# intel/neural-compressor

Measured on AMD Instinct MI355X. Metric: llama2_7b_gptq_int4_g128_quantize_wall_clock, lower is better.
Workload: dtype bf16

## Files before the change

### include/inc_mi355x.h

```cpp
#ifndef INC_MI355X_H_
#define INC_MI355X_H_

#include <stdint.h>

#ifdef __cplusplus
extern "C" {
#endif

#define INC_OK 0
#define INC_ERR_BAD_ARG (-1)
#define INC_ERR_UNSUPPORTED (-2)
#define INC_ERR_LAUNCH (-3)
#define INC_ERR_WORKSPACE (-4)

#define INC_F32 0
#define INC_F16 1
#define INC_BF16 2

#define INC_SCHEME_ASYM 0
#define INC_SCHEME_SYM 1

typedef void* inc_stream_t;

int inc_abi_version(void);
// ... 184 lines not shown
                          inc_stream_t stream);
int inc_sq_weight_col_absmax(const void* w, int wdtype, int64_t N, int64_t K, float* out, inc_stream_t stream);
int inc_sq_cal_scale(const float* amax_x, const float* amax_w, int64_t K, float alpha, float weight_max_lb, float* scale,
                     inc_stream_t stream);
int inc_sq_quant_weight(const void* w, int wdtype, int64_t N, int64_t K, int64_t Kp, const float* smooth, int8_t* qw,
                        float* w_scale, int32_t* rowsum, inc_stream_t stream);
int inc_sq_quant_act(const void* x, int xdtype, int64_t M, int64_t K, int64_t Kp, const float* in_scale, float sx, float zp,
                     int8_t* out, inc_stream_t stream);
int inc_w8a8_gemm(const int8_t* xq, const int8_t* wq, const float* alpha, const int32_t* corr, const void* bias, void* y,
                  int ydtype, int64_t M, int64_t N, int64_t K, void* workspace, int64_t workspace_bytes,
                  inc_stream_t stream);
int inc_sq_quant_act_token(const void* x, int xdtype, int64_t M, int64_t K, int64_t Kp, const float* in_scale, int8_t* xq,
                           float* row_scale, inc_stream_t stream);
int inc_w8a8_gemm_rowscale(const int8_t* xq, const int8_t* wq, const float* row_scale, const float* alpha, const void* bias,
                           void* y, int ydtype, int64_t M, int64_t N, int64_t K, void* workspace, int64_t workspace_bytes,
                           inc_stream_t stream);

#define INC_MX_FP8_E4M3 0
#define INC_MX_FP4_E2M1 4
#define INC_MX_KTILE 128
#define INC_MX_GEMV_MAX_M 16
int inc_mx_quant(const void* x, int xdtype, int64_t M, int64_t K, int64_t Kp, int fmt, uint8_t* codes, uint8_t* scales,
                 inc_stream_t stream);
int inc_mx_gemm(const uint8_t* xq, const uint8_t* xs, int xfmt, const uint8_t* wq, const uint8_t* ws, int wfmt, const void* bias,
                void* y, int ydtype, int64_t M, int64_t N, int64_t Kp, inc_stream_t stream);
int inc_mx_gemv(const uint8_t* xq, const uint8_t* xs, int xfmt, const uint8_t* wq, const uint8_t* ws, int wfmt, const void* bias,
                void* y, int ydtype, int64_t M, int64_t N, int64_t Kp, inc_stream_t stream);
int inc_mx_gemv_multi(int n, const uint8_t* xq, const uint8_t* xs, int xfmt, const uint8_t* const* wq, const uint8_t* const* ws,
                      int wfmt, const void* const* bias, void* const* y, int ydtype, int64_t M, const int64_t* N, int64_t Kp,
                      inc_stream_t stream);
int inc_mx_moe_gemm(int mode, const uint8_t* aq, const uint8_t* as, int afmt, const int32_t* route, const uint8_t* wq,
                    const uint8_t* ws, int wfmt, const void* routing_weights, int wdtype, void* out, int odtype, int64_t T, int top_k,
                    int64_t E, int64_t N, int64_t Kp, inc_stream_t stream);

int inc_fp8_quant_rows(const void* x, int xdtype, int64_t M, int64_t K, int64_t Kp, const float* in_scale, uint8_t* codes,
                       float* row_scale, inc_stream_t stream);
int inc_fp8_gemm(const uint8_t* xq, const float* row_scale, const uint8_t* wq, const float* alpha, const void* bias, void* y, int ydtype,
                 int64_t M, int64_t N, int64_t Kp, inc_stream_t stream);
int inc_fp8_gemv(const uint8_t* xq, const float* row_scale, const uint8_t* wq, const float* alpha, const void* bias, void* y, int ydtype,
                 int64_t M, int64_t N, int64_t Kp, inc_stream_t stream);
int inc_fp8_moe_gemm(int mode, const uint8_t* aq, const float* a_scale, const int32_t* route, const uint8_t* wq, const float* alpha,
                     const void* routing_weights, int wdtype, void* out, int odtype, int64_t T, int top_k, int64_t E, int64_t N,
                     int64_t Kp, inc_stream_t stream);

int inc_probe_hbm_triad(float* a, const float* b, const float* c, float s, int64_t n, inc_stream_t stream);
int inc_probe_hbm_copy(void* dst, const void* src, int64_t bytes, int variant, inc_stream_t stream);
int inc_probe_mfma_bf16(const void* src, float* sink, int blocks, int iters, double* flops_out, inc_stream_t stream);
int inc_trace_marker(int id, inc_stream_t stream);

int inc_fwd_silu_mul(const void* gate, const void* up, void* out, int64_t n, int dtype, inc_stream_t stream);
int inc_fwd_rope(const void* q, const void* k, const void* cos, const void* sin, void* q_out, void* k_out, int64_t B, int64_t Hq,
                 int64_t Hk, int64_t T, int64_t D, const int64_t* strides, int64_t cs_batch, int dtype, inc_stream_t stream);
int inc_fwd_rmsnorm(const void* x, const void* w, void* out, int64_t rows, int64_t cols, float eps, int dtype, inc_stream_t stream);

#ifdef __cplusplus
}
#endif
#endif
```

### neural_compressor_amd/_lib.py

```python

import ctypes
import os
from ctypes import c_char_p, c_float, c_int, c_int64, c_void_p

_HERE = os.path.dirname(os.path.abspath(__file__))
LIB_PATH = os.path.join(_HERE, "libinc_mi355x.so")
ABI_VERSION = 12

INC_OK = 0
INC_F32, INC_F16, INC_BF16 = 0, 1, 2
INC_SCHEME_ASYM, INC_SCHEME_SYM = 0, 1

_P = c_void_p
SIGNATURES = {
    "inc_abi_version": (c_int, []),
    "inc_error_string": (c_char_p, [c_int]),
    "inc_target_arch": (c_char_p, []),
    "inc_pack_rows": (c_int, [_P, _P, c_int64, c_int64, c_int, c_int, _P]),
    "inc_unpack_rows": (c_int, [_P, _P, c_int64, c_int64, c_int, c_int, c_int, _P]),
    "inc_woq_pack": (c_int, [_P, c_int, _P, _P, _P, _P, _P, c_int64, c_int64, c_int64, c_int, c_int, _P]),
    "inc_woq_unpack": (c_int, [_P, _P, _P, _P, c_int64, c_int64, c_int64, c_int, _P, _P, _P]),
    "inc_woq_dequant": (c_int, [_P, _P, _P, _P, _P, c_int, c_int64, c_int64, c_int64, c_int, c_int, _P]),
    "inc_dequant_ints": (c_int, [_P, _P, c_int, _P, _P, _P, c_int, c_int64, c_int64, c_int64, c_int, _P]),
    "inc_woq_gemm_workspace_bytes": (c_int64, [c_int64, c_int64, c_int64]),
# ... 53 lines not shown
    "inc_gptq_find_params": (
        c_int,
        [_P, c_int64, c_int64, c_int64, c_int, c_int, c_int, c_int, _P, _P, c_int64, c_int64, _P],
    ),
    "inc_sq_channel_minmax": (c_int, [_P, c_int, c_int64, c_int64, c_int64, _P, _P, _P]),
    "inc_sq_weight_col_absmax": (c_int, [_P, c_int, c_int64, c_int64, _P, _P]),
    "inc_sq_cal_scale": (c_int, [_P, _P, c_int64, c_float, c_float, _P, _P]),
    "inc_sq_quant_weight": (c_int, [_P, c_int, c_int64, c_int64, c_int64, _P, _P, _P, _P, _P]),
    "inc_sq_quant_act": (c_int, [_P, c_int, c_int64, c_int64, c_int64, _P, c_float, c_float, _P, _P]),
    "inc_w8a8_gemm_workspace_bytes": (c_int64, [c_int64, c_int64, c_int64]),
    "inc_w8a8_gemm": (c_int, [_P, _P, _P, _P, _P, _P, c_int, c_int64, c_int64, c_int64, _P, c_int64, _P]),
    "inc_sq_quant_act_token": (c_int, [_P, c_int, c_int64, c_int64, c_int64, _P, _P, _P, _P]),
    "inc_w8a8_gemm_rowscale": (c_int, [_P, _P, _P, _P, _P, _P, c_int, c_int64, c_int64, c_int64, _P, c_int64, _P]),
    "inc_mx_quant": (c_int, [_P, c_int, c_int64, c_int64, c_int64, c_int, _P, _P, _P]),
    "inc_mx_gemm": (c_int, [_P, _P, c_int, _P, _P, c_int, _P, _P, c_int, c_int64, c_int64, c_int64, _P]),
    "inc_mx_gemv": (c_int, [_P, _P, c_int, _P, _P, c_int, _P, _P, c_int, c_int64, c_int64, c_int64, _P]),
    "inc_mx_gemv_multi": (c_int, [c_int, _P, _P, c_int, _P, _P, c_int, _P, _P, c_int, c_int64, _P, c_int64, _P]),
    "inc_mx_moe_gemm": (
        c_int,
        [c_int, _P, _P, c_int, _P, _P, _P, c_int, _P, c_int, _P, c_int, c_int64, c_int, c_int64, c_int64, c_int64, _P],
    ),
    "inc_fp8_quant_rows": (c_int, [_P, c_int, c_int64, c_int64, c_int64, _P, _P, _P, _P]),
    "inc_fp8_gemm": (c_int, [_P, _P, _P, _P, _P, _P, c_int, c_int64, c_int64, c_int64, _P]),
    "inc_fp8_gemv": (c_int, [_P, _P, _P, _P, _P, _P, c_int, c_int64, c_int64, c_int64, _P]),
    "inc_fp8_moe_gemm": (
        c_int,
        [c_int, _P, _P, _P, _P, _P, _P, c_int, _P, c_int, c_int64, c_int, c_int64, c_int64, c_int64, _P],
    ),
    "inc_awq_repack": (c_int, [_P, _P, c_int64, c_int64, c_int64, c_int, _P, _P, _P]),
    "inc_gptq_find_params_mse": (
        c_int,
        [_P, c_int64, c_int64, c_int64, c_int, c_int, c_int, c_int, c_int, c_float, c_float, _P, _P, c_int64, c_int64, _P],
    ),
    "inc_gptq_quant_block": (
        c_int,
        [_P, _P, _P, _P, _P, _P, c_int, _P, c_int64, c_int64, c_int64, c_int64, c_int, c_int, c_int, _P],
    ),
    "inc_gptq_quant_block_params": (c_int, [_P, _P, _P, _P, _P, _P, c_int, _P, c_int64, c_int64, c_int64, c_int64, c_int, c_int, c_int, c_int, _P]),
    "inc_gptq_lazy_update": (c_int, [_P, _P, _P, c_int64, c_int64, c_int64, c_int, _P]),
    "inc_gptq_lazy_update_cols": (c_int, [_P, _P, _P, c_int64, c_int64, c_int64, c_int, c_int64, c_int64, _P]),
    "inc_probe_hbm_triad": (c_int, [_P, _P, _P, c_float, c_int64, _P]),
    "inc_probe_hbm_copy": (c_int, [_P, _P, c_int64, c_int, _P]),
    "inc_probe_mfma_bf16": (c_int, [_P, _P, c_int, c_int, _P, _P]),
    "inc_trace_marker": (c_int, [c_int, _P]),
    "inc_gptq_quantize_layer": (c_int, [_P, _P, _P, _P, c_int64, _P, _P, c_int64, _P, _P, c_int, _P, c_int64, c_int64, c_int, c_int, c_int,
                                        c_int, c_int, c_int, _P, _P]),
    "inc_chol_diag_block": (c_int, [_P, c_int64, c_int, _P, c_int64, _P, c_int, _P]),
    "inc_gptq_inverse_factor_workspace_bytes": (c_int64, [c_int64, c_int]),
    "inc_gptq_inverse_factor": (c_int, [_P, c_int64, _P, _P, c_int64, _P, c_int, _P, _P]),
    "inc_awq_act_abs_sum": (c_int, [_P, c_int, c_int64, c_int64, _P, _P]),
    "inc_awq_weight_scale_workspace_bytes": (c_int64, [c_int64, c_int64, c_int]),
    "inc_awq_weight_scale": (c_int, [_P, c_int, c_int64, c_int64, c_int, _P, _P, c_int64, _P]),
    "inc_fwd_silu_mul": (c_int, [_P, _P, _P, c_int64, c_int, _P]),
    "inc_fwd_rope": (c_int, [_P, _P, _P, _P, _P, _P, c_int64, c_int64, c_int64, c_int64, c_int64, _P, c_int64, c_int, _P]),
    "inc_fwd_rmsnorm": (c_int, [_P, _P, _P, c_int64, c_int64, c_float, c_int, _P]),
}


class IncLibraryError(RuntimeError):
    """Raised when libinc_mi355x.so is missing, stale, or a call returns an INC_ERR_* code."""


def _load():
    if not os.path.exists(LIB_PATH):
        raise IncLibraryError(
            f"{LIB_PATH} not found. The MI355X HIP extension is mandatory (there is no CPU fallback): "
            "build it with `python -c 'import __graft_entry__ as g; g.build()'` or "
            "`make -C neural_compressor_amd/csrc`."
        )
    lib = ctypes.CDLL(LIB_PATH)
    for name, (restype, argtypes) in SIGNATURES.items():
        try:
            fn = getattr(lib, name)
        except AttributeError as e:
            raise IncLibraryError(f"{LIB_PATH} does not export `{name}`; rebuild the extension") from e
        fn.restype = restype
        fn.argtypes = argtypes
    got = lib.inc_abi_version()
    if got != ABI_VERSION:
        raise IncLibraryError(f"ABI mismatch: library reports {got}, bindings expect {ABI_VERSION}; rebuild")
    return lib


lib = _load()


def check(code, what):
    if code != INC_OK:
        msg = lib.inc_error_string(code).decode()
        raise IncLibraryError(f"{what} failed: {msg} (code {code})")
```

### neural_compressor_amd/csrc/fwd_elementwise.hip

```cpp
#include "common.hpp"

namespace {

typedef uint32_t u32x4 __attribute__((ext_vector_type(4)));

template <int DT>
__device__ __forceinline__ uint16_t t_round(float f) {
  if constexpr (DT == INC_BF16) {
    uint32_t u = __float_as_uint(f);
    if ((u & 0x7fffffffu) > 0x7f800000u) return 0x7FC0;
    u += 0x7fffu + ((u >> 16) & 1u);
    return static_cast<uint16_t>(u >> 16);
  } else {
    return f32_to_f16_bits(f);
  }
}
template <int DT>
__device__ __forceinline__ float t_f32(uint16_t b) {
  if constexpr (DT == INC_BF16) return bf16_bits_to_f32(b);
  else return f16_bits_to_f32(b);
}
template <int DT>
__device__ __forceinline__ float t_rf(float f) { return t_f32<DT>(t_round<DT>(f)); }

template <int DT>
__device__ __forceinline__ void unpack8(const u32x4 v, float (&e)[8]) {
#pragma unroll
  for (int i = 0; i < 4; ++i) {
    e[2 * i] = t_f32<DT>(static_cast<uint16_t>(v[i] & 0xffffu));
    e[2 * i + 1] = t_f32<DT>(static_cast<uint16_t>(v[i] >> 16));
  }
}
__device__ __forceinline__ u32x4 pack8(const uint16_t (&b)[8]) {
  u32x4 v;
#pragma unroll
  for (int i = 0; i < 4; ++i) v[i] = static_cast<uint32_t>(b[2 * i]) | (static_cast<uint32_t>(b[2 * i + 1]) << 16);
  return v;
}
__device__ __forceinline__ u32x4 ld_nt(const void* p, int64_t i16) { return __builtin_nontemporal_load(static_cast<const u32x4*>(p) + i16); }
__device__ __forceinline__ void st_nt(void* p, int64_t i16, u32x4 v) { __builtin_nontemporal_store(v, static_cast<u32x4*>(p) + i16); }

template <int DT>
__device__ __forceinline__ uint16_t silu_mul_one(float g, float u) {
#pragma clang fp contract(off)
  const float s = t_rf<DT>(g / (1.0f + expf(-g)));
  return t_round<DT>(s * u);
}

template <int DT>
__global__ __launch_bounds__(256) void fwd_silu_mul_kernel(const void* __restrict__ gate, const void* __restrict__ up, void* __restrict__ out, int64_t n) {
  const int64_t n8 = n >> 3;
  const int64_t i = (int64_t)blockIdx.x * 256 + threadIdx.x;
  if (i < n8) {
    float g[8], u[8];
    unpack8<DT>(ld_nt(gate, i), g);
    unpack8<DT>(ld_nt(up, i), u);
    uint16_t r[8];
#pragma unroll
    for (int e = 0; e < 8; ++e) r[e] = silu_mul_one<DT>(g[e], u[e]);
    st_nt(out, i, pack8(r));
  } else {
    const int64_t e = n8 * 8 + (i - n8);
    if (e < n) {
      const uint16_t* g = static_cast<const uint16_t*>(gate);
      const uint16_t* u = static_cast<const uint16_t*>(up);
      static_cast<uint16_t*>(out)[e] = silu_mul_one<DT>(t_f32<DT>(g[e]), t_f32<DT>(u[e]));
    }
  }
}

struct RopeStrides {
  int64_t q[3], k[3], qo[3], ko[3];
};

template <int DT>
__global__ __launch_bounds__(256) void fwd_rope_kernel(const void* __restrict__ q, const void* __restrict__ k, const void* __restrict__ cosp,
                                                       const void* __restrict__ sinp, void* __restrict__ q_out, void* __restrict__ k_out,
                                                       uint32_t total, uint32_t Hq, uint32_t Hk, uint32_t T, uint32_t D, uint32_t cs_batch,
                                                       RopeStrides st) {
#pragma clang fp contract(off)
  const uint32_t idx = blockIdx.x * 256u + threadIdx.x;
  if (idx >= total) return;
  const uint32_t d16 = D >> 4, H = Hq + Hk;
  const uint32_t dc = idx % d16;
  uint32_t r = idx / d16;
  const uint32_t hh = r % H;
  r /= H;
  const uint32_t t = r % T, b = r / T;
  const bool is_k = hh >= Hq;
  const uint32_t h = is_k ? hh - Hq : hh;
  const int64_t* si = is_k ? st.k : st.q;
  const int64_t* so = is_k ? st.ko : st.qo;
  const char* src = static_cast<const char*>(is_k ? k : q);
  char* dst = static_cast<char*>(is_k ? k_out : q_out);
  const int64_t in_off = (int64_t)b * si[0] + (int64_t)h * si[1] + (int64_t)t * si[2] + dc * 8;
  const int64_t out_off = (int64_t)b * so[0] + (int64_t)h * so[1] + (int64_t)t * so[2] + dc * 8;
  const int64_t cs_off = ((int64_t)(cs_batch == 1 ? 0 : b) * T + t) * D + dc * 8;
  const int64_t half = D >> 1;

  float lo[8], hi[8], c_lo[8], c_hi[8], s_lo[8], s_hi[8];
  unpack8<DT>(ld_nt(src, in_off >> 3), lo);
  unpack8<DT>(ld_nt(src, (in_off + half) >> 3), hi);
  unpack8<DT>(static_cast<const u32x4*>(cosp)[cs_off >> 3], c_lo);
  unpack8<DT>(static_cast<const u32x4*>(cosp)[(cs_off + half) >> 3], c_hi);
  unpack8<DT>(static_cast<const u32x4*>(sinp)[cs_off >> 3], s_lo);
  unpack8<DT>(static_cast<const u32x4*>(sinp)[(cs_off + half) >> 3], s_hi);
  uint16_t o_lo[8], o_hi[8];
#pragma unroll
  for (int e = 0; e < 8; ++e) {
    o_lo[e] = t_round<DT>(t_rf<DT>(lo[e] * c_lo[e]) + t_rf<DT>(-hi[e] * s_lo[e]));
    o_hi[e] = t_round<DT>(t_rf<DT>(hi[e] * c_hi[e]) + t_rf<DT>(lo[e] * s_hi[e]));
  }
  st_nt(dst, out_off >> 3, pack8(o_lo));
  st_nt(dst, (out_off + half) >> 3, pack8(o_hi));
}

template <int DT, int WAVES, int J>
__global__ __launch_bounds__(WAVES == 1 ? 256 : 512) void fwd_rmsnorm_kernel(const void* __restrict__ x, const void* __restrict__ w, void* __restrict__ out,
                                                                              int64_t rows, int cols, float eps, float factor) {
#pragma clang fp contract(off)
  constexpr int HALVES = (WAVES == 1 ? 256 : 512) / 32, ROWS_PER_BLOCK = HALVES / WAVES;
  __shared__ float part[ROWS_PER_BLOCK][8];
  const int p = threadIdx.x & 31, hw = threadIdx.x >> 5;
  const int rb = hw / WAVES, tw = hw % WAVES;
  const int64_t row = (int64_t)blockIdx.x * ROWS_PER_BLOCK + rb;
  const bool live = row < rows;
  const int pieces = cols >> 3;
  const int64_t base = (live ? row : 0) * (int64_t)pieces;
  const int first = p + 32 * tw;

  u32x4 v[J];
#pragma unroll
  for (int j = 0; j < J; ++j) {
    const int u = first + 32 * WAVES * j;
    if (live && u < pieces) v[j] = ld_nt(x, base + u);
  }
  float a[4] = {0.f, 0.f, 0.f, 0.f}, b[4] = {0.f, 0.f, 0.f, 0.f};
#pragma unroll
  for (int j = 0; j < J; ++j) {
    const int u = first + 32 * WAVES * j;
    if (live && u < pieces) {
      float e[8];
      unpack8<DT>(v[j], e);
#pragma unroll
      for (int i = 0; i < 4; ++i) {
        a[i] = a[i] + e[i] * e[i];
        b[i] = b[i] + e[4 + i] * e[4 + i];
      }
    }
  }
  float s = (((a[0] + a[1]) + a[2]) + a[3]) + (((b[0] + b[1]) + b[2]) + b[3]);
#pragma unroll
  for (int o = 1; o < 32; o <<= 1) s = s + __shfl_down(s, o, 32);
  if constexpr (WAVES == 1) {
    s = __shfl(s, 0, 32);
  } else {
    if (p == 0) part[rb][tw] = s;
    __syncthreads();
    const float* q = part[rb];
    s = ((q[0] + q[4]) + (q[2] + q[6])) + ((q[1] + q[5]) + (q[3] + q[7]));
  }
  if (!live) return;
  const float mean = s * factor;
  const float rs = static_cast<float>(::rsqrt(static_cast<double>(mean + eps)));
#pragma unroll
  for (int j = 0; j < J; ++j) {
    const int u = first + 32 * WAVES * j;
    if (u < pieces) {
      float e[8], g[8];
      unpack8<DT>(v[j], e);
      unpack8<DT>(static_cast<const u32x4*>(w)[u], g);
      uint16_t r[8];
#pragma unroll
      for (int i = 0; i < 8; ++i) r[i] = t_round<DT>(g[i] * t_rf<DT>(e[i] * rs));
      st_nt(out, base + u, pack8(r));
    }
  }
}

template <int DT, int WAVES, int J>
void rmsnorm_launch(const void* x, const void* w, void* out, int64_t rows, int cols, float eps, float factor, hipStream_t s) {
  constexpr int THREADS = WAVES == 1 ? 256 : 512, ROWS_PER_BLOCK = THREADS / 32 / WAVES;
  fwd_rmsnorm_kernel<DT, WAVES, J><<<(unsigned)ceil_div64(rows, ROWS_PER_BLOCK), THREADS, 0, s>>>(x, w, out, rows, cols, eps, factor);
}

inline bool aligned16(const void* p) { return (reinterpret_cast<uintptr_t>(p) & 15u) == 0; }

}

extern "C" {

int inc_fwd_silu_mul(const void* gate, const void* up, void* out, int64_t n, int dtype, inc_stream_t stream) {
  INC_CHECK_ARG(gate && up && out && n > 0);
  if (dtype != INC_BF16 && dtype != INC_F16) return INC_ERR_UNSUPPORTED;
  if (!aligned16(gate) || !aligned16(up) || !aligned16(out)) return INC_ERR_UNSUPPORTED;
  const int64_t blocks = ceil_div64((n >> 3) + (n & 7), 256);
  if (blocks > 0x7fffffff) return INC_ERR_UNSUPPORTED;
  if (dtype == INC_BF16) fwd_silu_mul_kernel<INC_BF16><<<(unsigned)blocks, 256, 0, inc_s(stream)>>>(gate, up, out, n);
  else fwd_silu_mul_kernel<INC_F16><<<(unsigned)blocks, 256, 0, inc_s(stream)>>>(gate, up, out, n);
  INC_LAUNCH_RETURN();
}

int inc_fwd_rope(const void* q, const void* k, const void* cos, const void* sin, void* q_out, void* k_out, int64_t B, int64_t Hq,
                 int64_t Hk, int64_t T, int64_t D, const int64_t* strides, int64_t cs_batch, int dtype, inc_stream_t stream) {
  INC_CHECK_ARG(q && k && cos && sin && q_out && k_out && strides && B > 0 && Hq > 0 && Hk > 0 && T > 0 && D > 0);
  INC_CHECK_ARG(cs_batch == 1 || cs_batch == B);
  if (dtype != INC_BF16 && dtype != INC_F16) return INC_ERR_UNSUPPORTED;
  if (D % 16 != 0) return INC_ERR_UNSUPPORTED;
  RopeStrides st;
  for (int i = 0; i < 3; ++i) {
    st.q[i] = strides[i];
    st.k[i] = strides[3 + i];
    st.qo[i] = strides[6 + i];
    st.ko[i] = strides[9 + i];
  }
  for (int i = 0; i < 12; ++i)
    if (strides[i] < 0 || strides[i] % 8 != 0) return INC_ERR_UNSUPPORTED;
  if (!aligned16(q) || !aligned16(k) || !aligned16(cos) || !aligned16(sin) || !aligned16(q_out) || !aligned16(k_out)) return INC_ERR_UNSUPPORTED;
  if (B >= (1ll << 31) || T >= (1ll << 31) || Hq + Hk >= (1ll << 31)) return INC_ERR_UNSUPPORTED;
  const double items = (double)B * (double)T * (double)(Hq + Hk) * (double)(D / 16);
  if (items >= 2147483648.0 - 256.0) return INC_ERR_UNSUPPORTED;
  const uint32_t total = (uint32_t)(B * T * (Hq + Hk) * (D / 16));
  const unsigned blocks = (total + 255u) / 256u;
  if (dtype == INC_BF16)
    fwd_rope_kernel<INC_BF16><<<blocks, 256, 0, inc_s(stream)>>>(q, k, cos, sin, q_out, k_out, total, (uint32_t)Hq, (uint32_t)Hk, (uint32_t)T, (uint32_t)D, (uint32_t)cs_batch, st);
  else
    fwd_rope_kernel<INC_F16><<<blocks, 256, 0, inc_s(stream)>>>(q, k, cos, sin, q_out, k_out, total, (uint32_t)Hq, (uint32_t)Hk, (uint32_t)T, (uint32_t)D, (uint32_t)cs_batch, st);
  INC_LAUNCH_RETURN();
}

int inc_fwd_rmsnorm(const void* x, const void* w, void* out, int64_t rows, int64_t cols, float eps, int dtype, inc_stream_t stream) {
  INC_CHECK_ARG(x && w && out && rows > 0 && cols > 0);
  if (dtype != INC_BF16 && dtype != INC_F16) return INC_ERR_UNSUPPORTED;
  if (rows < 8 || cols % 8 != 0 || cols < 256 || cols > 16384 || rows >= (1ll << 40)) return INC_ERR_UNSUPPORTED;
  if (!aligned16(x) || !aligned16(w) || !aligned16(out)) return INC_ERR_UNSUPPORTED;
  if (ceil_div64(rows, 2) > 0x7fffffff) return INC_ERR_UNSUPPORTED;
  const float factor = static_cast<float>(rows) / static_cast<float>(rows * cols);
  const int c = (int)cols;
  hipStream_t s = inc_s(stream);
#define INC_RMS(W, JJ)                                                                        \
  do {                                                                                        \
    if (dtype == INC_BF16) rmsnorm_launch<INC_BF16, W, JJ>(x, w, out, rows, c, eps, factor, s); \
    else rmsnorm_launch<INC_F16, W, JJ>(x, w, out, rows, c, eps, factor, s);                    \
  } while (0)
  if (cols <= 8128) {
    if (cols <= 2048) INC_RMS(1, 8);
    else if (cols <= 4096) INC_RMS(1, 16);
    else if (cols <= 6144) INC_RMS(1, 24);
    else INC_RMS(1, 32);
  } else {
    INC_RMS(8, 8);
  }
#undef INC_RMS
  INC_LAUNCH_RETURN();
}

}
```

### neural_compressor_amd/ops.py

```python

import torch

from ._lib import INC_BF16, INC_F16, INC_F32, INC_SCHEME_ASYM, INC_SCHEME_SYM, check, lib

_DT = {torch.float32: INC_F32, torch.float16: INC_F16, torch.bfloat16: INC_BF16}


def dtype_code(dtype):
    try:
        return _DT[dtype]
    except KeyError as e:
        raise TypeError(f"unsupported floating dtype {dtype}; expected fp32/fp16/bf16") from e


def _dev(*tensors):
    dev = None
    for t in tensors:
        if t is None:
            continue
        if t.device.type != "cuda":
            raise RuntimeError(
                f"MI355X op got a tensor on {t.device}; tensors must be resident in HBM (device 'cuda' = HIP). "
                "There is no CPU fallback."
            )
# ... 1091 lines not shown
def _fwd_call(fn, name, args):
    rc = fn(*args)
    if rc == -2:
        return False
    check(rc, name)
    return True


def fwd_silu_mul(gate, up):
    dev = _dev(gate, up)
    if gate.shape != up.shape or gate.dtype != up.dtype or gate.numel() == 0:
        return None
    out = torch.empty_like(gate)
    with torch.cuda.device(dev):
        ok = _fwd_call(lib.inc_fwd_silu_mul, "inc_fwd_silu_mul", (_ptr(gate), _ptr(up), _ptr(out), gate.numel(), dtype_code(gate.dtype), _stream()))
    return out if ok else None


def fwd_rmsnorm(x, weight, eps):
    dev = _dev(x, weight)
    cols = x.shape[-1]
    if x.dtype != weight.dtype or weight.shape != (cols,) or x.numel() == 0:
        return None
    out = torch.empty_like(x)
    with torch.cuda.device(dev):
        ok = _fwd_call(lib.inc_fwd_rmsnorm, "inc_fwd_rmsnorm",
                       (_ptr(x), _ptr(weight), _ptr(out), x.numel() // cols, cols, float(eps), dtype_code(x.dtype), _stream()))
    return out if ok else None


def fwd_rope(q, k, cos, sin, q_out_strides, k_out_strides):
    import ctypes

    for t in (q, k, cos, sin):
        if t.device.type != "cuda" or t.device != q.device or t.dtype != q.dtype:
            return None
    if q.dim() != 4 or k.dim() != 4 or cos.dim() != 3 or cos.shape != sin.shape or not cos.is_contiguous() or not sin.is_contiguous():
        return None
    B, Hq, T, D = q.shape
    if k.shape[0] != B or k.shape[2] != T or k.shape[3] != D or cos.shape[1:] != (T, D) or cos.shape[0] not in (1, B):
        return None
    if q.numel() == 0 or k.numel() == 0 or q.stride(3) != 1 or k.stride(3) != 1 or q_out_strides[3] != 1 or k_out_strides[3] != 1:
        return None
    q_out = torch.empty_strided(q.shape, q_out_strides, dtype=q.dtype, device=q.device)
    k_out = torch.empty_strided(k.shape, k_out_strides, dtype=k.dtype, device=k.device)
    strides = (ctypes.c_int64 * 12)(*q.stride()[:3], *k.stride()[:3], *q_out_strides[:3], *k_out_strides[:3])
    with torch.cuda.device(q.device):
        ok = _fwd_call(lib.inc_fwd_rope, "inc_fwd_rope",
                       (_ptr(q), _ptr(k), _ptr(cos), _ptr(sin), _ptr(q_out), _ptr(k_out), B, Hq, k.shape[1], T, D, strides, cos.shape[0],
                        dtype_code(q.dtype), _stream()))
    return (q_out, k_out) if ok else None


_HIP_RT = None


def cu_masked_stream(device, mask_words):
    global _HIP_RT
    import ctypes

    try:
        if _HIP_RT is None:
            _HIP_RT = ctypes.CDLL("libamdhip64.so")
        st = ctypes.c_void_p()
        arr = (ctypes.c_uint32 * len(mask_words))(*mask_words)
        with torch.cuda.device(device):
            if _HIP_RT.hipExtStreamCreateWithCUMask(ctypes.byref(st), len(mask_words), arr) != 0 or not st.value:
                return None
            return torch.cuda.ExternalStream(st.value, device=device)
    except Exception:
        return None


def trace_marker(marker_id, device=None):
    with torch.cuda.device(device if device is not None else torch.cuda.current_device()):
        check(lib.inc_trace_marker(int(marker_id), _stream()), "inc_trace_marker")


GPTQ_DYNAMIC_GROUPS, GPTQ_MSE, GPTQ_NO_LOOKAHEAD, GPTQ_NO_FUSED_PARAMS = 1, 2, 4, 8


def gptq_quantize_layer(w32, hinv, scale, zero, loop_scale, loop_zero, codes, q_out, err_ws, group_size, kernel_group_size, block_size,
                        bits, sym, flags, aux_stream=None):
    dev = _dev(w32, hinv, scale, zero, codes, q_out, err_ws)
    N, K = w32.shape
    assert err_ws.dtype == torch.float32 and err_ws.numel() >= 2 * N * 128
    with torch.cuda.device(dev):
        check(
            lib.inc_gptq_quantize_layer(
                _ptr(w32), _ptr(hinv), _ptr(scale), _ptr(zero), scale.shape[1], _ptr(loop_scale), _ptr(loop_zero),
                loop_scale.shape[1] if loop_scale is not None else scale.shape[1], _ptr(codes), _ptr(q_out),
                dtype_code(q_out.dtype) if q_out is not None else INC_F32, _ptr(err_ws), N, K, int(group_size), int(kernel_group_size),
                int(block_size), int(bits), 1 if sym else 0, int(flags), _stream(),
                aux_stream.cuda_stream if aux_stream is not None else None,
            ),
            "inc_gptq_quantize_layer",
        )


def chol_diag_block(A_view, Linv_view, info, tag):
    dev = A_view.device
    if dev.type != "cuda" or Linv_view.device != dev:
        raise RuntimeError("chol_diag_block needs HBM-resident views")
    n = A_view.shape[0]
    assert A_view.shape == (n, n) and Linv_view.shape == (n, n) and A_view.stride(1) == 1 and Linv_view.stride(1) == 1
    assert A_view.dtype == torch.float32 and Linv_view.dtype == torch.float32
# ... 321 lines not shown
```

### neural_compressor_amd/torch/algorithms/weight_only/gptq.py

```python

import math
import os
import time
from functools import partial

import torch
import torch.nn as nn

from .... import ops
from ....common.utils import logger
from ...utils.utility import batch_broadcastable, get_accelerator, get_model_device, set_module
from ..base_algorithm import Quantizer as INCQuantizer
from .fused_forward import FusedForward
from .modules import MI355XWeightOnlyLinear

try:
    import transformers

    _Conv1D = transformers.Conv1D
    SUPPORTED_LAYERS = (nn.Linear, transformers.Conv1D)
except Exception:
    _Conv1D = None
    SUPPORTED_LAYERS = (nn.Linear,)

# ... 468 lines not shown
            codes = codes[:, invperm].contiguous()
            inv_global = torch.argsort(torch.div(perm.reshape(G, gs)[:, 0], gs, rounding_mode="floor"))
            scale = scale[:, inv_global].contiguous()
            zero = zero[:, inv_global].contiguous()
        self.codes = codes
        self.export_perm = None if (static_groups or not act_order) else self.perm
        if self.is_conv1d:
            Q = Q.t().contiguous()
        Q = Q.reshape(weight_shape)
        if not self.defer_check:
            self.acc.check()
        return scale, torch.tensor([-1]), zero, Q

    def free(self):
        self.acc = None
        self.codes = None


def _to_device(obj, device):
    if isinstance(obj, torch.Tensor):
        return obj.to(device)
    if isinstance(obj, (list, tuple)):
        return type(obj)(_to_device(o, device) for o in obj)
    if isinstance(obj, dict):
        return {k: _to_device(v, device) for k, v in obj.items()}
    return obj


class RAWGPTQuantizer(object):

    def __init__(self, model, weight_config={}, nsamples=128, use_max_length=True, max_seq_length=2048, device=None,
                 use_layer_wise=False, model_path="", quant_lm_head=False, dataloader=None, use_block_wise=False,
                 *args, **kwargs):
        self.model = model
        self.gptq_related_blocks = trace_gptq_target_blocks(self.model)
        self.dtype = next(iter(self.model.parameters())).dtype
        self.weight_config = weight_config
        self.quant_lm_head = quant_lm_head
        self.check_layer_config()
        self.device = torch.device(get_accelerator(device or "auto").current_device_name())
        self.is_ready = False
        self.use_layer_wise = False
        self.use_block_wise = False
        self.use_max_length = use_max_length
        self.max_seq_length = max_seq_length
        self.nsamples = nsamples
        self.share_hessians = kwargs.get("share_hessians", True)
        self.factor_streams = int(os.environ.get("INC_MI355X_GPTQ_FACTOR_STREAMS", "4"))
        self._fstreams = []
        self._late_stream = None
        self._block_writes_input = None
        self._fused = FusedForward()
        self._stacks = {}
        self.block_callback = kwargs.get("block_callback", None)
        self.hessian_allreduce = kwargs.get("hessian_allreduce", None)
        self.row_shard_solve = kwargs.get("row_shard_solve", None)
        self.solve_2d = kwargs.get("solve_2d", SOLVE_2D)
        mode = os.environ.get("INC_MI355X_GPTQ_MULTI_GPU", "")
        if mode and (self.hessian_allreduce is None and self.row_shard_solve is None):
            import torch.distributed as dist

            from ....distributed import live as _dist_live

            live = _dist_live()
            assert mode in ("sample", "rows", "sample+rows", "layer"), f"INC_MI355X_GPTQ_MULTI_GPU={mode!r}"
            self.hessian_allreduce = live and mode in ("sample", "sample+rows")
            self.row_shard_solve = live and mode in ("rows", "sample+rows")
            if mode == "layer" and kwargs.get("independent_blocks") is None:
                kwargs["independent_blocks"] = True
        self.independent_blocks = kwargs.get("independent_blocks", None)
        self.layer_ctx = None
        if self.independent_blocks:
            import torch.distributed as dist

            assert not (self.hessian_allreduce or self.row_shard_solve), "independent_blocks excludes the sample / rows modes"
            if dist.is_available() and dist.is_initialized():
                from ....distributed import SINGLE_RANK_GROUP, CalibrationGroup

                ctx = CalibrationGroup(None if self.independent_blocks is True else self.independent_blocks)
                self.layer_ctx = ctx if (ctx.world > 1 or SINGLE_RANK_GROUP) else None
        self.dist_ctx = None
        if self.row_shard_solve:
            from ....distributed import SINGLE_RANK_GROUP, CalibrationGroup

            self.dist_ctx = CalibrationGroup(None if self.row_shard_solve is True else self.row_shard_solve)
            if self.dist_ctx.world == 1 and not SINGLE_RANK_GROUP:
                self.dist_ctx = None

    _DEFAULTS = dict(
        dtype="int", bits=4, group_size=128, block_size=128, percdamp=0.01, sym=False, act_order=False,
        hybrid_order=False, fp8_aware=False, static_groups=False, true_sequential=False, perchannel=True, mse=False,
        use_double_quant=False, double_quant_dtype="int", double_quant_bits=4, double_quant_group_size=128,
        double_quant_sym=False,
    )

    def check_layer_config(self):
        for layer_name, config in self.weight_config.items():
            for key, default in self._DEFAULTS.items():
                config[key] = config.get(key, default)
            if config["dtype"] != "int" and "int" in config["dtype"]:
                config["bits"] = int(config["dtype"].lstrip("int"))
                config["dtype"] = "int"

    def get_layer_config(self, layer_name):
        import re

# ... 621 lines not shown
        handle.remove()
        if self.dist_ctx is not None:
            self._exchange_factors([(solver.acc, cfg["percdamp"], cfg["act_order"])])
            solver.row_ctx = self.dist_ctx
        elif self.hessian_allreduce:
            solver.acc.allreduce(None if self.hessian_allreduce is True else self.hessian_allreduce)
        elif self.layer_ctx is not None and self.layer_ctx.world > 1:
            solver.acc.allreduce(self.layer_ctx.group)
        scale, _, zp, Q = solver.fasterquant(
            layer.weight.data, blocksize=cfg["block_size"], percdamp=cfg["percdamp"], groupsize=cfg["group_size"],
            act_order=cfg["act_order"], hybrid_order=cfg["hybrid_order"], fp8_aware=cfg["fp8_aware"],
            static_groups=cfg["static_groups"],
        )
        if isinstance(layer, nn.Linear):
            in_features, out_features = layer.in_features, layer.out_features
        else:
            in_features, out_features = layer.weight.shape[0], layer.weight.shape[1]
        zero = None if cfg["sym"] else zp
        new_module = MI355XWeightOnlyLinear(
            in_features, out_features, dtype=cfg["dtype"], bits=cfg["bits"], group_size=cfg["group_size"],
            zp=zero is not None, bias=layer.bias is not None, g_idx=solver.export_perm is not None, device=self.device,
        )
        new_module.pack_codes(solver.codes, scale, zero, layer.bias, g_idx=solver.export_perm)
        solver.acc.check()
        solver.free()
        set_module(self.model, full, new_module)

    @torch.no_grad()
    def quantize_block(self, block, block_idx, seq_map=None, propagate=True):
        sub_layers = find_layers(block)
        from .experts_gptq import quantize_block_experts

        quantize_block_experts(self, block, block_idx)
        sequentials = seq_map if seq_map else [list(sub_layers.keys())]
        for sequential in sequentials:
            layers = {}
            for name in sequential:
                full = self.get_full_layer_name(name, block_idx)
                if self.get_layer_config(full) is None:
                    logger.warning("%s can be quantized but excluded from quantization configs.", full)
                else:
                    layers[name] = sub_layers[name]
            solvers = {}
            for name, layer in layers.items():
                solvers[name] = GPTQ(layer, device=self.device)
                solvers[name].defer_check = True
                solvers[name].configure(self.get_layer_config(self.get_full_layer_name(name, block_idx)))
                cfg_ = solvers[name].cfg
                if cfg_.get("hybrid_order", False):
                    GPTQ.check_hybrid_order(solvers[name].columns, cfg_.get("group_size", -1), cfg_.get("act_order", False), cfg_.get("static_groups", False))
            live, alias = {}, {}
            share = self.share_hessians

            fired, seen, capture = [], set(), {"probe": True, "stop": None}

            def make_hook(name):
                def body(inp):
                    x = inp[0].detach()
                    key = (x.data_ptr(), tuple(x.shape), x.dtype, x._version)
                    if share and key in live:
                        owner = live[key][0]
                        if alias.setdefault(name, owner) != owner:
                            raise RuntimeError(f"{name}: input sharing changed between calibration batches")
                        return
                    if alias.get(name) is not None:
                        raise RuntimeError(f"{name}: input sharing changed between calibration batches")
                    live[key] = (name, x)
                    solvers[name].add_batch(x)

                def hook(_, inp):
                    if capture["probe"]:
                        fired.append(name)
                    seen.add(name)
                    body(inp)
                    if capture["stop"] == name and len(seen) == len(layers):
                        raise _CaptureDone

                return hook

            handles = [layers[n].register_forward_pre_hook(make_hook(n)) for n in layers]
            accs = [sv.acc for sv in solvers.values()]
            for acc in accs:
                acc.defer = True

            def after_forward(j, out):
                live.clear()
                seen.clear()
                HessianAccumulator.flush_many(accs, only_due=True)
                if capture["probe"]:
                    capture["probe"] = False
                    if CAPTURE_EARLY_STOP and len(fired) == len(layers) and set(fired) == set(layers):
                        capture["stop"] = fired[-1]

            with _phase("gptq.capture_forward"):
                self._run_block(block, on_output=after_forward, capture=True)
                HessianAccumulator.flush_many(accs)
            for acc in accs:
                acc.defer = False
            for h in handles:
                h.remove()
            def hybrid_gs(sv):
                if not sv.cfg.get("hybrid_order", False):
                    return 0
                gs_ = sv.cfg.get("group_size", -1)
                return sv.columns if (gs_ == -1 or gs_ >= sv.columns) else int(gs_)

            for name, owner in alias.items():
                if (
                    solvers[name].columns == solvers[owner].columns
                    and solvers[name].cfg["percdamp"] == solvers[owner].cfg["percdamp"]
                    and solvers[name].cfg["act_order"] == solvers[owner].cfg["act_order"]
                    and hybrid_gs(solvers[name]) == hybrid_gs(solvers[owner])
                ):
                    solvers[name].acc = solvers[owner].acc
                else:
                    raise RuntimeError(f"{name} shares its input with {owner} but not its GPTQ settings; pass share_hessians=False")
            distinct, seen = [], set()
            for name in layers:
                acc = solvers[name].acc
                if id(acc) not in seen:
                    seen.add(id(acc))
                    distinct.append((acc, solvers[name].cfg["percdamp"], solvers[name].cfg["act_order"], hybrid_gs(solvers[name])))
            _KEYS = ("bits", "sym", "group_size", "block_size", "percdamp", "act_order", "hybrid_order", "fp8_aware",
                     "static_groups", "mse", "dtype", "use_double_quant")
            batches, index = [], {}
            for name, layer in layers.items():
                sv = solvers[name]
                key = None
                if isinstance(layer, nn.Linear) and self.share_hessians:
                    key = (id(sv.acc), layer.weight.dtype, tuple(sv.cfg.get(k) for k in _KEYS))
                if key is not None and key in index:
                    batches[index[key]].append(name)
                else:
                    if key is not None:
                        index[key] = len(batches)
                    batches.append([name])
            plan2d = None
            if self.dist_ctx is not None:
                plan2d = self._plan_2d(batches, solvers, distinct)
                if plan2d is not None:
                    self._exchange_factors_2d(plan2d, distinct)
                else:
                    self._exchange_factors(distinct)
                    for sv in solvers.values():
                        sv.row_ctx = self.dist_ctx
            elif self.hessian_allreduce:
                group = None if self.hessian_allreduce is True else self.hessian_allreduce
                for acc, _, _, _ in distinct:
                    acc.allreduce(group)
            if self.dist_ctx is None and len(distinct) > 1 and self.factor_streams > 1:
                if len(self._fstreams) < self.factor_streams:
                    self._fstreams = [torch.cuda.Stream(device=self.device) for _ in range(self.factor_streams)]
                order = sorted(range(len(distinct)), key=lambda i: -distinct[i][0].columns)
# ... 147 lines not shown
```

Measured before the change: 7.761.

## Cache capture hook order across blocks and vectorize bf16 rounding in elementwise kernels

The GPTQ capture loop now remembers, per block type, the order in which layer hooks fire and which accumulators passed the zero-copy check. Later blocks can then stop the capture forward early without a probe pass and skip re-validation. The elementwise forward kernels (silu_mul, rope, rmsnorm) switch to packed pair bf16 conversion with a NaN fallback, and rope gains a per-token walking kernel that loads cos/sin once and reuses them across heads. A probe_round16 entry point is added for testing rounding. The cached state risks going stale if blocks of the same type behave differently.

```diff
diff --git a/include/inc_mi355x.h b/include/inc_mi355x.h
--- a/include/inc_mi355x.h
+++ b/include/inc_mi355x.h
@@ -260,6 +260,7 @@
 int inc_fwd_rope(const void* q, const void* k, const void* cos, const void* sin, void* q_out, void* k_out, int64_t B, int64_t Hq,
                  int64_t Hk, int64_t T, int64_t D, const int64_t* strides, int64_t cs_batch, int dtype, inc_stream_t stream);
 int inc_fwd_rmsnorm(const void* x, const void* w, void* out, int64_t rows, int64_t cols, float eps, int dtype, inc_stream_t stream);
+int inc_probe_round16(const float* in, uint16_t* out, int64_t n, int dtype, inc_stream_t stream);
 
 #ifdef __cplusplus
 }
diff --git a/neural_compressor_amd/_lib.py b/neural_compressor_amd/_lib.py
--- a/neural_compressor_amd/_lib.py
+++ b/neural_compressor_amd/_lib.py
@@ -129,6 +129,7 @@
     "inc_awq_weight_scale_workspace_bytes": (c_int64, [c_int64, c_int64, c_int]),
     "inc_awq_weight_scale": (c_int, [_P, c_int, c_int64, c_int64, c_int, _P, _P, c_int64, _P]),
     "inc_fwd_silu_mul": (c_int, [_P, _P, _P, c_int64, c_int, _P]),
+    "inc_probe_round16": (c_int, [_P, _P, c_int64, c_int, _P]),
     "inc_fwd_rope": (c_int, [_P, _P, _P, _P, _P, _P, c_int64, c_int64, c_int64, c_int64, c_int64, _P, c_int64, c_int, _P]),
     "inc_fwd_rmsnorm": (c_int, [_P, _P, _P, c_int64, c_int64, c_float, c_int, _P]),
 }
diff --git a/neural_compressor_amd/csrc/fwd_elementwise.hip b/neural_compressor_amd/csrc/fwd_elementwise.hip
--- a/neural_compressor_amd/csrc/fwd_elementwise.hip
+++ b/neural_compressor_amd/csrc/fwd_elementwise.hip
@@ -24,18 +24,47 @@
 __device__ __forceinline__ float t_rf(float f) { return t_f32<DT>(t_round<DT>(f)); }
 
 template <int DT>
+__device__ __forceinline__ u32x4 round8(const float (&f)[8]) {
+  u32x4 v;
+  if constexpr (DT == INC_BF16) {
+    bool nan = false;
+#pragma unroll
+    for (int i = 0; i < 4; ++i) {
+      v[i] = cvt_pair<true>(f[2 * i], f[2 * i + 1]);
+      nan |= __builtin_isunordered(f[2 * i], f[2 * i + 1]);
+    }
+    if (__builtin_expect(nan, 0)) {
+#pragma unroll
+      for (int i = 0; i < 4; ++i) v[i] = static_cast<uint32_t>(t_round<DT>(f[2 * i])) | (static_cast<uint32_t>(t_round<DT>(f[2 * i + 1])) << 16);
+    }
+  } else {
+#pragma unroll
+    for (int i = 0; i < 4; ++i) v[i] = static_cast<uint32_t>(t_round<DT>(f[2 * i])) | (static_cast<uint32_t>(t_round<DT>(f[2 * i + 1])) << 16);
+  }
+  return v;
+}
+template <int DT>
+__device__ __forceinline__ void rf8(float (&f)[8]) {
+  if constexpr (DT == INC_BF16) {
+#pragma unroll
+    for (int i = 0; i < 4; ++i) {
+      const uint32_t r = cvt_pair<true>(f[2 * i], f[2 * i + 1]);
+      f[2 * i] = __uint_as_float(r << 16);
+      f[2 * i + 1] = __uint_as_float(r & 0xffff0000u);
+    }
+  } else {
+#pragma unroll
+    for (int i = 0; i < 8; ++i) f[i] = t_rf<DT>(f[i]);
+  }
+}
+
+template <int DT>
 __device__ __forceinline__ void unpack8(const u32x4 v, float (&e)[8]) {
 #pragma unroll
   for (int i = 0; i < 4; ++i) {
     e[2 * i] = t_f32<DT>(static_cast<uint16_t>(v[i] & 0xffffu));
     e[2 * i + 1] = t_f32<DT>(static_cast<uint16_t>(v[i] >> 16));
   }
-}
-__device__ __forceinline__ u32x4 pack8(const uint16_t (&b)[8]) {
-  u32x4 v;
-#pragma unroll
-  for (int i = 0; i < 4; ++i) v[i] = static_cast<uint32_t>(b[2 * i]) | (static_cast<uint32_t>(b[2 * i + 1]) << 16);
-  return v;
 }
 __device__ __forceinline__ u32x4 ld_nt(const void* p, int64_t i16) { return __builtin_nontemporal_load(static_cast<const u32x4*>(p) + i16); }
 __device__ __forceinline__ void st_nt(void* p, int64_t i16, u32x4 v) { __builtin_nontemporal_store(v, static_cast<u32x4*>(p) + i16); }
@@ -52,13 +81,16 @@
   const int64_t n8 = n >> 3;
   const int64_t i = (int64_t)blockIdx.x * 256 + threadIdx.x;
   if (i < n8) {
+#pragma clang fp contract(off)
     float g[8], u[8];
     unpack8<DT>(ld_nt(gate, i), g);
     unpack8<DT>(ld_nt(up, i), u);
-    uint16_t r[8];
-#pragma unroll
-    for (int e = 0; e < 8; ++e) r[e] = silu_mul_one<DT>(g[e], u[e]);
-    st_nt(out, i, pack8(r));
+#pragma unroll
+    for (int e = 0; e < 8; ++e) g[e] = g[e] / (1.0f + expf(-g[e]));
+    rf8<DT>(g);
+#pragma unroll
+    for (int e = 0; e < 8; ++e) g[e] = g[e] * u[e];
+    st_nt(out, i, round8<DT>(g));
   } else {
     const int64_t e = n8 * 8 + (i - n8);
     if (e < n) {
@@ -74,10 +106,106 @@
 };
 
 template <int DT>
+__device__ __forceinline__ void rope_pieces(const u32x4 v_lo, const u32x4 v_hi, const float (&c_lo)[8], const float (&c_hi)[8],
+                                            const float (&s_lo)[8], const float (&s_hi)[8], const uint32_t sign2, u32x4& o_lo, u32x4& o_hi) {
+#pragma clang fp contract(off)
+  float lo[8], hi[8], a[8], b[8];
+  unpack8<DT>(v_lo, lo);
+  unpack8<DT>(v_hi, hi);
+  if constexpr (DT == INC_BF16) {
+#pragma unroll
+    for (int e = 0; e < 8; ++e) b[e] = -hi[e];
+  } else {
+    u32x4 n_hi;
+#pragma unroll
+    for (int i = 0; i < 4; ++i) n_hi[i] = v_hi[i] ^ sign2;
+    unpack8<DT>(n_hi, b);
+  }
+#pragma unroll
+  for (int e = 0; e < 8; ++e) {
+    a[e] = lo[e] * c_lo[e];
+    b[e] = b[e] * s_lo[e];
+  }
+  rf8<DT>(a);
+  rf8<DT>(b);
+#pragma unroll
+  for (int e = 0; e < 8; ++e) a[e] = a[e] + b[e];
+  o_lo = round8<DT>(a);
+#pragma unroll
+  for (int e = 0; e < 8; ++e) {
+    a[e] = hi[e] * c_hi[e];
+    b[e] = lo[e] * s_hi[e];
+  }
+  rf8<DT>(a);
+  rf8<DT>(b);
+#pragma unroll
+  for (int e = 0; e < 8; ++e) a[e] = a[e] + b[e];
+  o_hi = round8<DT>(a);
+}
+
+constexpr int ROPE_WALK_U = 4;
+constexpr uint32_t ROPE_SIGN2 = 0x80008000u;
+
+template <int DT>
+__device__ __forceinline__ void rope_walk(const char* __restrict__ src, char* __restrict__ dst, const int64_t in_base, const int64_t out_base,
+                                          const int64_t in_hs, const int64_t out_hs, const uint32_t H, const uint32_t hsub, const uint32_t hpi,
+                                          const int64_t half, const float (&c_lo)[8], const float (&c_hi)[8], const float (&s_lo)[8],
+                                          const float (&s_hi)[8], const uint32_t sign2) {
+  for (uint32_t h0 = 0; h0 < H; h0 += hpi * ROPE_WALK_U) {
+    u32x4 v_lo[ROPE_WALK_U], v_hi[ROPE_WALK_U];
+#pragma unroll
+    for (int u = 0; u < ROPE_WALK_U; ++u) {
+      const uint32_t h = h0 + u * hpi + hsub;
+      if (h < H) {
+        const int64_t off = in_base + (int64_t)h * in_hs;
+        v_lo[u] = ld_nt(src, off >> 3);
+        v_hi[u] = ld_nt(src, (off + half) >> 3);
+      }
+    }
+#pragma unroll
+    for (int u = 0; u < ROPE_WALK_U; ++u) {
+      const uint32_t h = h0 + u * hpi + hsub;
+      if (h < H) {
+        u32x4 o_lo, o_hi;
+        rope_pieces<DT>(v_lo[u], v_hi[u], c_lo, c_hi, s_lo, s_hi, sign2, o_lo, o_hi);
+        const int64_t off = out_base + (int64_t)h * out_hs;
+        st_nt(dst, off >> 3, o_lo);
+        st_nt(dst, (off + half) >> 3, o_hi);
+      }
+    }
+  }
+}
+
+template <int DT>
+__global__ __launch_bounds__(256) void fwd_rope_walk_kernel(const void* __restrict__ q, const void* __restrict__ k, const void* __restrict__ cosp,
+                                                            const void* __restrict__ sinp, void* __restrict__ q_out, void* __restrict__ k_out,
+                                                            uint32_t tokens, uint32_t Hq, uint32_t Hk, uint32_t T, uint32_t D, uint32_t d16_log2,
+                                                            uint32_t cs_batch, uint32_t sign2, RopeStrides st) {
+  const uint32_t token = __builtin_amdgcn_readfirstlane(blockIdx.x * 4u + (threadIdx.x >> 6));
+  if (token >= tokens) return;
+  const uint32_t b = token / T, t = token - b * T;
+  const uint32_t lane = threadIdx.x & 63u;
+  const uint32_t dc = lane & ((1u << d16_log2) - 1u), hsub = lane >> d16_log2, hpi = 64u >> d16_log2;
+  const int64_t half = D >> 1;
+  const int64_t cs_off = ((int64_t)(cs_batch == 1 ? 0 : b) * T + t) * D + dc * 8;
+
+  float c_lo[8], c_hi[8], s_lo[8], s_hi[8];
+  unpack8<DT>(static_cast<const u32x4*>(cosp)[cs_off >> 3], c_lo);
+  unpack8<DT>(static_cast<const u32x4*>(cosp)[(cs_off + half) >> 3], c_hi);
+  unpack8<DT>(static_cast<const u32x4*>(sinp)[cs_off >> 3], s_lo);
+  unpack8<DT>(static_cast<const u32x4*>(sinp)[(cs_off + half) >> 3], s_hi);
+
+  rope_walk<DT>(static_cast<const char*>(q), static_cast<char*>(q_out), (int64_t)b * st.q[0] + (int64_t)t * st.q[2] + dc * 8,
+                (int64_t)b * st.qo[0] + (int64_t)t * st.qo[2] + dc * 8, st.q[1], st.qo[1], Hq, hsub, hpi, half, c_lo, c_hi, s_lo, s_hi, sign2);
+  rope_walk<DT>(static_cast<const char*>(k), static_cast<char*>(k_out), (int64_t)b * st.k[0] + (int64_t)t * st.k[2] + dc * 8,
+                (int64_t)b * st.ko[0] + (int64_t)t * st.ko[2] + dc * 8, st.k[1], st.ko[1], Hk, hsub, hpi, half, c_lo, c_hi, s_lo, s_hi, sign2);
+}
+
+template <int DT>
 __global__ __launch_bounds__(256) void fwd_rope_kernel(const void* __restrict__ q, const void* __restrict__ k, const void* __restrict__ cosp,
                                                        const void* __restrict__ sinp, void* __restrict__ q_out, void* __restrict__ k_out,
                                                        uint32_t total, uint32_t Hq, uint32_t Hk, uint32_t T, uint32_t D, uint32_t cs_batch,
-                                                       RopeStrides st) {
+                                                       uint32_t sign2, RopeStrides st) {
 #pragma clang fp contract(off)
   const uint32_t idx = blockIdx.x * 256u + threadIdx.x;
   if (idx >= total) return;
@@ -98,21 +226,16 @@
   const int64_t cs_off = ((int64_t)(cs_batch == 1 ? 0 : b) * T + t) * D + dc * 8;
   const int64_t half = D >> 1;
 
-  float lo[8], hi[8], c_lo[8], c_hi[8], s_lo[8], s_hi[8];
-  unpack8<DT>(ld_nt(src, in_off >> 3), lo);
-  unpack8<DT>(ld_nt(src, (in_off + half) >> 3), hi);
+  float c_lo[8], c_hi[8], s_lo[8], s_hi[8];
+  const u32x4 v_lo = ld_nt(src, in_off >> 3), v_hi = ld_nt(src, (in_off + half) >> 3);
   unpack8<DT>(static_cast<const u32x4*>(cosp)[cs_off >> 3], c_lo);
   unpack8<DT>(static_cast<const u32x4*>(cosp)[(cs_off + half) >> 3], c_hi);
   unpack8<DT>(static_cast<const u32x4*>(sinp)[cs_off >> 3], s_lo);
   unpack8<DT>(static_cast<const u32x4*>(sinp)[(cs_off + half) >> 3], s_hi);
-  uint16_t o_lo[8], o_hi[8];
-#pragma unroll
-  for (int e = 0; e < 8; ++e) {
-    o_lo[e] = t_round<DT>(t_rf<DT>(lo[e] * c_lo[e]) + t_rf<DT>(-hi[e] * s_lo[e]));
-    o_hi[e] = t_round<DT>(t_rf<DT>(hi[e] * c_hi[e]) + t_rf<DT>(lo[e] * s_hi[e]));
-  }
-  st_nt(dst, out_off >> 3, pack8(o_lo));
-  st_nt(dst, (out_off + half) >> 3, pack8(o_hi));
+  u32x4 o_lo, o_hi;
+  rope_pieces<DT>(v_lo, v_hi, c_lo, c_hi, s_lo, s_hi, sign2, o_lo, o_hi);
+  st_nt(dst, out_off >> 3, o_lo);
+  st_nt(dst, (out_off + half) >> 3, o_hi);
 }
 
 template <int DT, int WAVES, int J>
@@ -170,10 +293,12 @@
       float e[8], g[8];
       unpack8<DT>(v[j], e);
       unpack8<DT>(static_cast<const u32x4*>(w)[u], g);
-      uint16_t r[8];
-#pragma unroll
-      for (int i = 0; i < 8; ++i) r[i] = t_round<DT>(g[i] * t_rf<DT>(e[i] * rs));
-      st_nt(out, base + u, pack8(r));
+#pragma unroll
+      for (int i = 0; i < 8; ++i) e[i] = e[i] * rs;
+      rf8<DT>(e);
+#pragma unroll
+      for (int i = 0; i < 8; ++i) e[i] = g[i] * e[i];
+      st_nt(out, base + u, round8<DT>(e));
     }
   }
 }
@@ -182,6 +307,25 @@
 void rmsnorm_launch(const void* x, const void* w, void* out, int64_t rows, int cols, float eps, float factor, hipStream_t s) {
   constexpr int THREADS = WAVES == 1 ? 256 : 512, ROWS_PER_BLOCK = THREADS / 32 / WAVES;
   fwd_rmsnorm_kernel<DT, WAVES, J><<<(unsigned)ceil_div64(rows, ROWS_PER_BLOCK), THREADS, 0, s>>>(x, w, out, rows, cols, eps, factor);
+}
+
+template <int DT>
+__global__ __launch_bounds__(256) void probe_round16_kernel(const float* __restrict__ in, uint16_t* __restrict__ out, int64_t n) {
+  const int64_t n8 = n >> 3;
+  const int64_t i = (int64_t)blockIdx.x * 256 + threadIdx.x;
+  if (i < n8) {
+    const u32x4 a = static_cast<const u32x4*>(static_cast<const void*>(in))[2 * i], b = static_cast<const u32x4*>(static_cast<const void*>(in))[2 * i + 1];
+    float f[8];
+#pragma unroll
+    for (int e = 0; e < 4; ++e) {
+      f[e] = __uint_as_float(a[e]);
+      f[4 + e] = __uint_as_float(b[e]);
+    }
+    static_cast<u32x4*>(static_cast<void*>(out))[i] = round8<DT>(f);
+  } else {
+    const int64_t e = n8 * 8 + (i - n8);
+    if (e < n) out[e] = t_round<DT>(in[e]);
+  }
 }
 
 inline bool aligned16(const void* p) { return (reinterpret_cast<uintptr_t>(p) & 15u) == 0; }
@@ -220,12 +364,33 @@
   if (B >= (1ll << 31) || T >= (1ll << 31) || Hq + Hk >= (1ll << 31)) return INC_ERR_UNSUPPORTED;
   const double items = (double)B * (double)T * (double)(Hq + Hk) * (double)(D / 16);
   if (items >= 2147483648.0 - 256.0) return INC_ERR_UNSUPPORTED;
+  const uint32_t d16 = (uint32_t)(D / 16);
+  if ((d16 & (d16 - 1u)) == 0 && d16 <= 64u) {
+    const uint32_t tokens = (uint32_t)(B * T), lg = (uint32_t)__builtin_ctz(d16);
+    const unsigned wblocks = (tokens + 3u) / 4u;
+    if (dtype == INC_BF16)
+      fwd_rope_walk_kernel<INC_BF16><<<wblocks, 256, 0, inc_s(stream)>>>(q, k, cos, sin, q_out, k_out, tokens, (uint32_t)Hq, (uint32_t)Hk, (uint32_t)T, (uint32_t)D, lg, (uint32_t)cs_batch, ROPE_SIGN2, st);
+    else
+      fwd_rope_walk_kernel<INC_F16><<<wblocks, 256, 0, inc_s(stream)>>>(q, k, cos, sin, q_out, k_out, tokens, (uint32_t)Hq, (uint32_t)Hk, (uint32_t)T, (uint32_t)D, lg, (uint32_t)cs_batch, ROPE_SIGN2, st);
+    INC_LAUNCH_RETURN();
+  }
   const uint32_t total = (uint32_t)(B * T * (Hq + Hk) * (D / 16));
   const unsigned blocks = (total + 255u) / 256u;
   if (dtype == INC_BF16)
-    fwd_rope_kernel<INC_BF16><<<blocks, 256, 0, inc_s(stream)>>>(q, k, cos, sin, q_out, k_out, total, (uint32_t)Hq, (uint32_t)Hk, (uint32_t)T, (uint32_t)D, (uint32_t)cs_batch, st);
+    fwd_rope_kernel<INC_BF16><<<blocks, 256, 0, inc_s(stream)>>>(q, k, cos, sin, q_out, k_out, total, (uint32_t)Hq, (uint32_t)Hk, (uint32_t)T, (uint32_t)D, (uint32_t)cs_batch, ROPE_SIGN2, st);
   else
-    fwd_rope_kernel<INC_F16><<<blocks, 256, 0, inc_s(stream)>>>(q, k, cos, sin, q_out, k_out, total, (uint32_t)Hq, (uint32_t)Hk, (uint32_t)T, (uint32_t)D, (uint32_t)cs_batch, st);
+    fwd_rope_kernel<INC_F16><<<blocks, 256, 0, inc_s(stream)>>>(q, k, cos, sin, q_out, k_out, total, (uint32_t)Hq, (uint32_t)Hk, (uint32_t)T, (uint32_t)D, (uint32_t)cs_batch, ROPE_SIGN2, st);
+  INC_LAUNCH_RETURN();
+}
+
+int inc_probe_round16(const float* in, uint16_t* out, int64_t n, int dtype, inc_stream_t stream) {
+  INC_CHECK_ARG(in && out && n > 0);
+  if (dtype != INC_BF16 && dtype != INC_F16) return INC_ERR_UNSUPPORTED;
+  if (!aligned16(in) || !aligned16(out)) return INC_ERR_UNSUPPORTED;
+  const int64_t blocks = ceil_div64((n >> 3) + (n & 7), 256);
+  if (blocks > 0x7fffffff) return INC_ERR_UNSUPPORTED;
+  if (dtype == INC_BF16) probe_round16_kernel<INC_BF16><<<(unsigned)blocks, 256, 0, inc_s(stream)>>>(in, out, n);
+  else probe_round16_kernel<INC_F16><<<(unsigned)blocks, 256, 0, inc_s(stream)>>>(in, out, n);
   INC_LAUNCH_RETURN();
 }
 
diff --git a/neural_compressor_amd/ops.py b/neural_compressor_amd/ops.py
--- a/neural_compressor_amd/ops.py
+++ b/neural_compressor_amd/ops.py
@@ -1167,6 +1167,15 @@
     return (q_out, k_out) if ok else None
 
 
+def probe_round16(x, dtype):
+    dev = _dev(x)
+    assert x.dtype == torch.float32 and dtype in (torch.bfloat16, torch.float16)
+    out = torch.empty(x.shape, dtype=dtype, device=x.device)
+    with torch.cuda.device(dev):
+        check(lib.inc_probe_round16(_ptr(x), _ptr(out), x.numel(), dtype_code(dtype), _stream()), "inc_probe_round16")
+    return out
+
+
 _HIP_RT = None
 
 
diff --git a/neural_compressor_amd/torch/algorithms/weight_only/gptq.py b/neural_compressor_amd/torch/algorithms/weight_only/gptq.py
--- a/neural_compressor_amd/torch/algorithms/weight_only/gptq.py
+++ b/neural_compressor_amd/torch/algorithms/weight_only/gptq.py
@@ -544,6 +544,8 @@
         self._block_writes_input = None
         self._fused = FusedForward()
         self._stacks = {}
+        self._capture_order = {}
+        self._zero_copy_ok = set()
         self.block_callback = kwargs.get("block_callback", None)
         self.hessian_allreduce = kwargs.get("hessian_allreduce", None)
         self.row_shard_solve = kwargs.get("row_shard_solve", None)
@@ -1271,7 +1273,12 @@
             live, alias = {}, {}
             share = self.share_hessians
 
-            fired, seen, capture = [], set(), {"probe": True, "stop": None}
+            order_key = (type(block), tuple(layers))
+            remembered = self.__dict__.setdefault("_capture_order", {}).get(order_key) if CAPTURE_EARLY_STOP else None
+            if remembered is not None:
+                fired, seen, capture = list(remembered), set(), {"probe": False, "stop": remembered[-1], "stopped": False}
+            else:
+                fired, seen, capture = [], set(), {"probe": True, "stop": None, "stopped": False}
 
             def make_hook(name):
                 def body(inp):
@@ -1299,12 +1306,17 @@
 
             handles = [layers[n].register_forward_pre_hook(make_hook(n)) for n in layers]
             accs = [sv.acc for sv in solvers.values()]
-            for acc in accs:
-                acc.defer = True
+            zc_known = self.__dict__.setdefault("_zero_copy_ok", set())
+            for name, sv in solvers.items():
+                sv.acc.defer = True
+                if (type(block), name) in zc_known:
+                    sv.acc._zc_ok = True
 
             def after_forward(j, out):
                 live.clear()
                 seen.clear()
+                if out is None:
+                    capture["stopped"] = True
                 HessianAccumulator.flush_many(accs, only_due=True)
                 if capture["probe"]:
                     capture["probe"] = False
@@ -1318,6 +1330,13 @@
                 acc.defer = False
             for h in handles:
                 h.remove()
+            if remembered is not None:
+                if not capture["stopped"]:
+                    self._capture_order.pop(order_key, None)
+            elif capture["stop"] is not None:
+                self._capture_order[order_key] = tuple(fired)
+            zc_known.update((type(block), name) for name, sv in solvers.items() if sv.acc._zc_ok is True)
+
             def hybrid_gs(sv):
                 if not sv.cfg.get("hybrid_order", False):
                     return 0
```

New measurement: 7.511, median of 6. 1.03x faster.
